# maxall41/RustSASA

Hardware: AMD Instinct MI355X
Metric: structures/sec on AF2 E. coli proteome (100 pts, 1.4 A probe) (higher is better)
Workload: dtype f32

## Files before the change

### rustsasa_amd/csrc/context.cpp

```cpp
#include "engine_internal.h"

namespace rsasa {

const char *tuning_env(const char *name)
{
    static const bool on = [] { const char *v = std::getenv("RSASA_TUNING"); return v && std::atoi(v) != 0; }();
    return on ? std::getenv(name) : nullptr;
}

void generate_sphere_points(size_t n, float *x, float *y, float *z)
{
    const float pi = 3.14159274101257324219f;
    const float angle_increment = (2.0f * pi) * 1.618034f;
    const float inv_n = 1.0f / (float)n;
    for (size_t i = 0; i < n; i++) {
        const float fi = (float)i;
        const float t = fi * inv_n;
        const float inclination = acosf(1.0f - 2.0f * t);
        const float azimuth = angle_increment * fi;
        const float si = sinf(inclination);
        x[i] = si * cosf(azimuth);
        y[i] = si * sinf(azimuth);
        z[i] = cosf(inclination);
    }
// ... 284 lines not shown

int rsasa_context::Workspace::reserve_sorted(rsasa_context *ctx, size_t N, size_t cell_words, bool with_id)
{
    int rc;
    has_id = with_id;
    if ((rc = reserve(ctx, sid_sorted, std::max<size_t>(N, 1) * 4))) return rc;
    if ((rc = reserve(ctx, rank_of, std::max<size_t>(N, 1) * 4))) return rc;
    if ((rc = reserve(ctx, cells, cell_words * 4))) return rc;
    if ((rc = reserve(ctx, sorted_xyzr, std::max<size_t>(N, 1) * 16))) return rc;
    if ((rc = reserve(ctx, sorted_orig, std::max<size_t>(N, 1) * 4))) return rc;
    if (has_id && (rc = reserve(ctx, sorted_id32, std::max<size_t>(N, 1) * 4))) return rc;
    return RSASA_OK;
}

void rsasa_context::Workspace::sorted_view(BatchView &v) const
{
    v.sid_sorted = (uint32_t *)sid_sorted.p;
    v.cell_of = (uint32_t *)cell_of.p;
    v.rank_of = (uint32_t *)rank_of.p;
    v.cells = (uint32_t *)cells.p;
    v.sorted_xyzr = (float4 *)sorted_xyzr.p;
    v.sorted_orig = (uint32_t *)sorted_orig.p;
    v.sorted_id32 = has_id ? (uint32_t *)sorted_id32.p : nullptr;
}

int rsasa_context::Workspace::reserve_grid(rsasa_context *ctx, size_t N, size_t S, size_t n_seg_all, uint64_t &capacity, bool has_tail,
                                           bool with_id)
{
    int rc;
    if (capacity == 0) capacity = std::max<uint64_t>(1u << 16, 20ull * N + 512ull * S);
    capacity = std::min<uint64_t>(capacity, 0xFFFFFFF0ull);
    cell_capacity = capacity;
    window_capacity = (uint32_t)std::min<uint64_t>(2 * cell_capacity / kWindowCells + S + 1, 0x7FFFFFFFull);
    if ((rc = reserve(ctx, segments, std::max<size_t>(n_seg_all, 1) * sizeof(Segment)))) return rc;
    if ((rc = reserve(ctx, acc, std::max<size_t>(S, 1) * sizeof(StructAcc)))) return rc;
    if ((rc = reserve(ctx, grids, std::max<size_t>(S, 1) * sizeof(StructGrid)))) return rc;
    if ((rc = reserve(ctx, grid_sums, (std::max<size_t>(S, 1) + 255) / 256 * 32))) return rc;
    if (has_tail && (rc = reserve(ctx, cell_of, std::max<size_t>(N, 1) * 4))) return rc;
    if ((rc = reserve(ctx, windows, (size_t)window_capacity * sizeof(uint4)))) return rc;
    if ((rc = reserve(ctx, scan_sums, kScanBlocks * 4))) return rc;
    if ((rc = reserve(ctx, status, sizeof(BatchStatus)))) return rc;
    return reserve_sorted(ctx, N, (size_t)(cell_capacity + 1 + 3), with_id);
}

void rsasa_context::Workspace::grid_view(BatchView &v) const
{
    sorted_view(v);
    v.segments = (const Segment *)segments.p;
    v.acc = (StructAcc *)acc.p;
    v.grids = (StructGrid *)grids.p;
    v.grid_sums = (GridSums *)grid_sums.p;
    v.cell_capacity = cell_capacity;
    v.windows = (uint4 *)windows.p;
    v.window_capacity = window_capacity;
    v.scan_block_sums = (uint32_t *)scan_sums.p;
    v.status = (BatchStatus *)status.p;
}

int rsasa_context::Workspace::reserve_occlusion(rsasa_context *ctx, const Lattice &lat, size_t N, bool with_id, bool bitmaps,
                                                bool own_values)
{
    int rc;
    keep_ids = with_id && !occlusion_uses_mx(ctx->tuning, lat, (uint32_t)N);
    id_bitmaps = bitmaps;
    ids_seg_words = bitmaps ? (uint32_t)((N + 2047) / 2048) : 0u;
    own_atom_sasa = own_values;
    if ((rc = reserve(ctx, deferred_list, std::max<size_t>(N, 1) * 4))) return rc;
    if ((rc = reserve(ctx, claim, kClaimBytes))) return rc;
    if (id_bitmaps && (rc = reserve(ctx, ids_seg, 2 * (size_t)ids_seg_words * 4 + 16))) return rc;
    if (keep_ids && (rc = reserve(ctx, sorted_id, std::max<size_t>(N, 1) * 8))) return rc;
    if (own_atom_sasa && (rc = reserve(ctx, atom_sasa, std::max<size_t>(N, 1) * 4))) return rc;
    return RSASA_OK;
}

void rsasa_context::Workspace::occlusion_view(BatchView &v) const
{
    v.deferred_list = (uint32_t *)deferred_list.p;
    v.claim = (uint32_t *)claim.p;
    v.ids_seg = id_bitmaps ? (uint32_t *)ids_seg.p : nullptr;
    v.ids_seg_words = ids_seg_words;
    v.sorted_id = keep_ids ? (uint64_t *)sorted_id.p : nullptr;
    if (own_atom_sasa) v.atom_sasa = (float *)atom_sasa.p;
}

namespace rsasa {

int grid_input_error(rsasa_context *ctx, const BatchStatus &stt)
// ... 37 lines not shown
    if (n_seg_all * sizeof(Segment) > hs.h_segments.cap) {
        if (hs.h_segments.p) RS_HIP(ctx, hipStreamSynchronize(pd.stream));
        RS_HIP(ctx, hs.h_segments.regrow((n_seg_all + n_seg_all / 2 + 64) * sizeof(Segment)));
    }
    Segment *h_segments = static_cast<Segment *>(hs.h_segments.p);
    write_segments(bt.structure_offsets_host, S, h_segments, reinterpret_cast<uint32_t *>(h_segments + n_seg));

    const bool has_id = bt.id != nullptr;
    if ((rc = W.reserve_grid(ctx, N, S, n_seg_all, ctx->cell_capacity, has_tail, has_id))) return rc;
    if ((rc = W.reserve_occlusion(ctx, lat, N, has_id, has_id, !bt.out_atom_sasa))) return rc;
    const bool keep_ids = W.keep_ids;
    if (keep_ids && pd.id32) return fail(ctx, RSASA_ERR_INTERNAL, "folded ids on a batch the per-atom kernels take");

    if (n_seg_all)
        RS_HIP(ctx, hipMemcpyAsync(W.segments.p, h_segments, n_seg_all * sizeof(Segment),
                                   hipMemcpyHostToDevice, st));

    BatchView v{};
    v.x = bt.x; v.y = bt.y; v.z = bt.z; v.radius = bt.radius; v.id = bt.id;
    v.id32 = pd.id32;
    v.ids_check = (has_id && !pd.ids_needed_known && !keep_ids && !tuning_env("RSASA_NO_ID_CHECK")) ? 1u : 0u;
    hs.ids_check = v.ids_check != 0u;
    v.large_sids = reinterpret_cast<const uint32_t *>((const Segment *)W.segments.p + n_seg);
    v.n_large = (uint32_t)n_large;
    v.ids_tables = ctx->ids_unordered_hint ? 1u : 0u;
    v.radius8 = pd.radius8;
    v.radius_table = pd.radius_table;
    v.residue_offsets = bt.residue_offsets;
    v.n_atoms = (uint32_t)N; v.n_structures = (uint32_t)S; v.n_residues = (uint32_t)R;
    v.n_segments = (uint32_t)n_seg;
    v.probe = pd.probe;
    v.atom_sasa = bt.out_atom_sasa;
    W.grid_view(v);
    W.occlusion_view(v);
    v.residue_sasa = (R && bt.residue_offsets) ? bt.out_residue_sasa : nullptr;
    v.neighbor_counts = bt.out_neighbor_counts;

    if (ctx->timing) RS_HIP(ctx, hipEventRecord(W.ev[0], st));
    launch_grid_prepare(v, st);
    rsasa_context::Workspace &other = ctx->ws[pd.ws ^ 1];
    const bool chain = other.occ_recorded && !tuning_env("RSASA_FREE_OVERLAP");
    const bool overlap = ctx->overlap_tail && has_tail;
    if (overlap && (rc = ensure_side_stream(ctx))) return rc;
    if (overlap) {
        launch_sort_lds(v, st);
        RS_HIP(ctx, hipEventRecord(ctx->ev_fork, st));
        RS_HIP(ctx, hipStreamWaitEvent(ctx->side_stream, ctx->ev_fork, 0));
        launch_sort_tail(v, ctx->side_stream);
        RS_HIP(ctx, hipEventRecord(ctx->ev_join, ctx->side_stream));
        if (ctx->timing) RS_HIP(ctx, hipEventRecord(W.ev[1], st));
        if (chain) RS_HIP(ctx, hipStreamWaitEvent(st, other.ev_occ, 0));
        if (ctx->timing) RS_HIP(ctx, hipEventRecord(W.ev[2], st));
        launch_occlusion(v, lat, ctx->tuning, kOccHead, st);
        RS_HIP(ctx, hipStreamWaitEvent(st, ctx->ev_join, 0));
        launch_occlusion(v, lat, ctx->tuning, kOccRest, st);
    } else {
        launch_sort_lds(v, st);
        if (has_tail) launch_sort_tail(v, st);
        if (ctx->timing) RS_HIP(ctx, hipEventRecord(W.ev[1], st));
        OcclusionChain oc;
        oc.wait = chain ? other.ev_occ : nullptr;
        oc.start = ctx->timing ? W.ev[2] : nullptr;
        oc.done = W.ev_occ;
        oc.expect_ids_dropped = ctx->ids_drop_hint;
        oc.solo = pd.solo_ok && v.ids_check != 0u;
        launch_occlusion(v, lat, ctx->tuning, kOccAll, st, &oc);
// ... 3 lines not shown
    if (ctx->timing) RS_HIP(ctx, hipEventRecord(W.ev[3], st));
    launch_residue_sums(v, st);
    if (ctx->timing) RS_HIP(ctx, hipEventRecord(W.ev[4], st));
    RS_HIP(ctx, hipMemcpyAsync(hs.h_status.p, W.status.p, sizeof(BatchStatus),
                               hipMemcpyDeviceToHost, st));
    RS_HIP(ctx, hipGetLastError());
    return RSASA_OK;
}

int wait_one(rsasa_context *ctx, Pending &pd)
{
    if (!pd.active) return RSASA_OK;
    rsasa_context::Workspace &W = ctx->ws[pd.ws];
    for (;;) {
        hipError_t e = hipStreamSynchronize(pd.stream);
        if (e != hipSuccess) {
            pd.active = false;
            return fail(ctx, RSASA_ERR_HIP, "hipStreamSynchronize", e);
        }
        const BatchStatus stt = ctx->slot[pd.ws].status();
        int rc = grid_verdict(ctx, stt, pd.attempts, ctx->cell_capacity);
        const bool solo_missed = rc == RSASA_OK && ctx->slot[pd.ws].ids_check && (stt.ids_unordered & 2u) != 0u;
        if (rc == kGridAgain) {
            pd.attempts++;
        } else if (solo_missed && pd.solo_ok) {
            ctx->ids_drop_hint = false;
            ctx->ids_unordered_hint = (stt.ids_unordered & 1u) != 0u;
            pd.solo_ok = false;
        } else {
            if (solo_missed) {
                rc = fail(ctx, RSASA_ERR_INTERNAL, "a launch pair reports the id-less launch's verdict");
            } else if (rc == RSASA_OK) {
                ctx->tuning.deferred_hint = stt.deferred;
                if (ctx->slot[pd.ws].ids_check) {
                    ctx->ids_drop_hint = !stt.ids_needed;
                    ctx->ids_unordered_hint = (stt.ids_unordered & 1u) != 0u;
                    ctx->ids_kept_structures.store(stt.ids_needed, std::memory_order_relaxed);
                    if (!stt.ids_needed) ctx->ids_dropped.fetch_add(1, std::memory_order_relaxed);
                }
                if (ctx->timing) {
                    float g = 0, o = 0, a = 0, t = 0;
                    (void)hipEventElapsedTime(&g, W.ev[0], W.ev[1]);
                    (void)hipEventElapsedTime(&o, W.ev[2], W.ev[3]);
                    (void)hipEventElapsedTime(&a, W.ev[3], W.ev[4]);
                    (void)hipEventElapsedTime(&t, W.ev[0], W.ev[4]);
                    ctx->timings = rsasa_timings_t{g, o, a, t, stt.grid_cells, pd.batch.n_atoms, stt.deferred};
                    ctx->timings_valid = true;
                }
            }
            pd.active = false;
            return rc;
        }
        if ((rc = enqueue_batch(ctx, pd, ctx->slot[pd.ws]))) {
            pd.active = false;
            return rc;
        }
    }
}

int wait_oldest(rsasa_context *ctx)
{
    if (ctx->n_pending == 0) return RSASA_OK;
    const int rc = wait_one(ctx, ctx->pending[ctx->head]);
    ctx->head ^= 1;
    ctx->n_pending--;
    return rc;
// ... 388 lines not shown
```

### rustsasa_amd/csrc/device_types.h

```cpp
#pragma once
#include <hip/hip_runtime.h>
#include <stdint.h>

namespace rsasa {

struct StructGrid {
    float min_x, min_y, min_z;
    float inv_cell;
    uint32_t dim_x, dim_y, dim_z;
    uint32_t cell_base;
    float max_r;
    float cell_size;
    uint32_t n_cells;
    uint32_t atom_begin;
    uint32_t n_atoms;
    uint32_t sorted_base;
    uint32_t in_lds;
    uint32_t odd_radii;
};
static_assert(sizeof(StructGrid) == 64, "StructGrid layout");

struct StructAcc {
    int min_x, min_y, min_z;
    int max_x, max_y, max_z;
// ... 41 lines not shown
inline uint32_t mx_tab_tiles(uint32_t n_points) { return n_points <= 96u ? 6u : n_points <= 112u ? 7u : 8u; }
inline uint32_t mx_tab_floats(uint32_t n_points) { return n_points > 128u ? 0u : 4u * (16u * mx_tab_tiles(n_points) + 16u) + 2u * 16u * mx_tab_tiles(n_points); }

struct GridSums {
    unsigned long long cells_s, cells_l, atoms_s, atoms_l;
};

struct BatchView {
    const float *x, *y, *z, *radius;
    const uint64_t *id;
    const uint32_t *id32;
    const uint8_t *radius8;
    const float *radius_table;
    const uint32_t *residue_offsets;
    uint32_t n_atoms, n_structures, n_residues, n_segments;
    float probe;
    uint32_t ids_check;
    const uint32_t *large_sids;
    uint32_t n_large;
    uint32_t ids_tables;
    const Segment *segments;
    StructAcc *acc;
    StructGrid *grids;
    uint32_t *sid_sorted;
    uint32_t *cell_of, *rank_of;
    uint32_t *deferred_list;
    uint32_t *claim;
    uint32_t *ids_seg;
    uint32_t ids_seg_words;
    uint32_t *cells;
    uint64_t cell_capacity;
    uint4 *windows;
    uint32_t window_capacity;
    uint32_t *scan_block_sums;
    GridSums *grid_sums;
    float4 *sorted_xyzr;
    uint32_t *sorted_orig;
    uint64_t *sorted_id;
    uint32_t *sorted_id32;
    BatchStatus *status;
    float *atom_sasa;
    float *residue_sasa;
    uint32_t *neighbor_counts;
    uint32_t *defer_flag;
    float max_r_override = __builtin_nanf("");
};

struct NbInfo {
    unsigned long long total;
    unsigned long long max_k;
    unsigned long long spill_entries;
    unsigned long long spill_atoms;
    unsigned long long spill_cursor;
    unsigned long long spill_recs;
    unsigned long long mismatch;
    unsigned long long pad;
};
static_assert(sizeof(NbInfo) == 64, "NbInfo layout");
struct NbKey {
    unsigned long long key;
    float thr;
    uint32_t pad;
};
struct NbSpillRec {
    unsigned long long off, base;
    uint32_t k, pad;
// ... 64 lines not shown
    kOccHead = 1,
    kOccRest = 2,
};
struct OcclusionChain {
    hipEvent_t wait = nullptr, start = nullptr, done = nullptr;
    bool expect_ids_dropped = true;
    bool solo = false;
};
void launch_occlusion(const BatchView &b, const Lattice &lat, const OcclusionTuning &tune,
                      OcclusionPart part, hipStream_t stream, const OcclusionChain *chain = nullptr);
bool occlusion_uses_mx(const OcclusionTuning &tune, const Lattice &lat, uint32_t n_atoms);
void launch_occlusion_deferred(const BatchView &b, const Lattice &lat, hipStream_t stream);
void launch_residue_sums(const BatchView &b, hipStream_t stream);
void launch_neighbor_count(const NbArgs &a, hipStream_t stream);
void launch_neighbor_fill(const NbArgs &a, uint64_t spill_atoms, hipStream_t stream);
void launch_accessible_points(const PtArgs &a, hipStream_t stream);
void launch_exposure_vectors(const ExArgs &e, hipStream_t stream);
void launch_contact_points(const CtArgs &c, hipStream_t stream);
void launch_neighbor_scan(const NbArgs &a, hipStream_t stream);
void launch_group_order(const GpArgs &g, hipStream_t stream);
void launch_group_points(const GpArgs &g, hipStream_t stream);
void launch_unpack_atoms(const void *records, uint32_t n_atoms, float *x, float *y, float *z, float *r, uint64_t *id,
                         const void *hdr_src, void *hdr_dst, uint32_t hdr_bytes, hipStream_t stream);
void launch_expand_frames(const float *xyz, const float *radius, const uint64_t *id,
                          const uint32_t *res_off, uint32_t n_atoms, uint32_t n_frames, uint32_t res_stride,
                          float *x, float *y, float *z, float *r, uint64_t *id_out,
                          uint32_t *res_out, hipStream_t stream);

constexpr uint32_t kSegmentAtoms = 4096;
constexpr uint32_t kScanBlocks = 1024;
constexpr uint32_t kWindowCells = 36864;
constexpr uint32_t kIdSlotsSmall = 8192, kIdAtomsSmall = 4096, kIdSlotsLarge = 73728, kIdAtomsLarge = 55296;
constexpr uint32_t kLdsMaxAtoms = 65536;

__host__ __device__ inline uint32_t grid_group_shift(uint32_t n_atoms, uint32_t n_cells)
{
    const float per_cell = (float)n_atoms / (float)(n_cells ? n_cells : 1u);
    return per_cell >= 1.0f ? 0u : per_cell >= 0.6f ? 1u : per_cell >= 0.3f ? 2u : 3u;
}
__host__ __device__ constexpr uint32_t lds_cell_slots(uint32_t n_cells) { return (n_cells + 1u + 7u) & ~7u; }
__host__ __device__ constexpr uint32_t grid_windows(uint32_t n_cells) { return (n_cells + kWindowCells - 1u) / kWindowCells; }

}
```

### rustsasa_amd/csrc/engine_internal.h

```cpp
#pragma once
#include "../../include/rustsasa_amd.h"

#include <hip/hip_runtime.h>

#include <algorithm>
#include <chrono>
#include <atomic>
#include <cmath>
#include <cstdio>
#include <cstdlib>
#include <cstring>
#include <condition_variable>
#include <deque>
#include <map>
#include <memory>
#include <mutex>
#include <thread>
#include <new>
#include <string>
#include <utility>
#include <vector>

#include <pthread.h>
#include <sched.h>
// ... 269 lines not shown
    uint64_t next_ticket = 1;
    LinkGate gate;
    bool quit = false;
};

}

using namespace rsasa;

struct rsasa_context {
    int device = 0;
    NodeCpus node;
    Stream stream;
    std::recursive_mutex mu;
    std::string last_error;
    int simd_width = 8;
    bool timing = false;
    bool small_path = true;
    bool overlap_tail = false;
    Stream side_stream;
    Event ev_fork, ev_join;
    rsasa_timings_t timings{};
    bool timings_valid = false;

    struct Workspace {
        DeviceBuffer segments, acc, grids, grid_sums, sid_sorted, deferred_list, cell_of, rank_of, cells, windows, scan_sums,
            sorted_xyzr, sorted_orig, sorted_id, sorted_id32, status, atom_sasa, claim, ids_seg;
        Event ev[5];
        Event ev_occ;
        bool occ_recorded = false;
        uint64_t cell_capacity = 0;
        uint32_t window_capacity = 0, ids_seg_words = 0;
        bool has_id = false, keep_ids = false, id_bitmaps = false, own_atom_sasa = false;

        int reserve_sorted(rsasa_context *ctx, size_t N, size_t cell_words, bool has_id);
        void sorted_view(BatchView &v) const;
        int reserve_grid(rsasa_context *ctx, size_t N, size_t S, size_t n_seg_all, uint64_t &cell_capacity, bool has_tail, bool has_id);
        void grid_view(BatchView &v) const;
        int reserve_occlusion(rsasa_context *ctx, const Lattice &lat, size_t N, bool has_id, bool id_bitmaps, bool own_atom_sasa);
        void occlusion_view(BatchView &v) const;
    } ws[2];
    static constexpr int kInFlight = 2;
    Stream stream2;
    DeviceBuffer in_x, in_y, in_z, in_r, in_id, in_res, out_res, out_k;
    static constexpr int kSlots = 8;
    struct MoreSlot { DeviceBuffer x, y, z, r, id, res, atom_sasa, out_res; } more[kSlots - 1];
    DeviceBuffer in_pack[kSlots];
    PinnedBlock h_pack;
    FoldPool *fold_pool = nullptr;
    RadiusCodec radius_codec;
    Stream copy_stream;
    Stream d2h_stream;
    Event ev_copy[kSlots];
    Event ev_d2h[kSlots];
    PinnedBlock h_out[kSlots];
    DeviceBuffer small_in, small_out;
    PinnedBlock h_small;
    DeviceBuffer tr_xyz, tr_r, tr_id, tr_res;
    struct HostSlot {
        PinnedBlock h_segments;
        PinnedBlock h_status;
        PinnedBlock h_res;
        const BatchStatus &status() const { return *static_cast<const BatchStatus *>(h_status.p); }
        bool ids_check = false;
    } slot[kSlots];
    std::atomic<uint64_t> ids_dropped{0};
    std::atomic<uint64_t> ids_kept_structures{0};
    bool ids_drop_hint = true;
    bool ids_unordered_hint = false;
    Event ev_done[kSlots];
    uint64_t cell_capacity = 0;

    std::map<std::pair<size_t, int>, LatticeEntry> lattices;
    Pending pending[2];
    int head = 0, n_pending = 0;
    OcclusionTuning tuning;
    Event ev_link;
    Event tr_ev[8][4];
    LinkGate *link_gate = nullptr;
    uint64_t link_ticket = 0;
    int own_queues = 0;
    size_t stream_sub_batches = 0;
    struct HostStream *host_stream = nullptr;
    std::atomic<int> combine_wait_us{-1};
    Workspace nb_ws;
    DeviceBuffer nb_x, nb_y, nb_z, nb_r, nb_id, nb_map, nb_counts, nb_offsets, nb_parts, nb_info, nb_entries, nb_spill, nb_recs;
    PinnedBlock nb_host;
    uint64_t nb_cell_capacity = 0;
    DeviceBuffer pt_masks, pt_sasa, pt_lattice;
    size_t pt_lattice_points = 0;
    DeviceBuffer ex_vectors, ex_free;
    DeviceBuffer ct_covered, ct_exclusive;
    DeviceBuffer gp_group, gp_sorted, gp_sorted_group, gp_own, gp_nrows, gp_offsets, gp_groups, gp_buried, gp_only, gp_self_free,
        gp_free;
};

namespace rsasa {

int fail(rsasa_context *ctx, int code, const char *what, hipError_t e = hipSuccess);

struct DeviceGuard {
// ... 129 lines not shown
```

### rustsasa_amd/csrc/host_batch.cpp

```cpp
#include "engine_internal.h"

namespace {

bool small_grid(const float mn_in[3], const float mx_in[3], float max_r, float probe, uint32_t n_atoms,
                StructGrid *out)
{
    const float cell = probe + max_r;
    const float inv = 1.0f / cell;
    if (!(cell > 0.0f) || !(inv < INFINITY) || !(cell < INFINITY)) return false;
    StructGrid g{};
    unsigned long long nc = 1;
    uint32_t d[3];
    const float mn[3] = {mn_in[0] - cell, mn_in[1] - cell, mn_in[2] - cell};
    const float mx[3] = {mx_in[0] + cell, mx_in[1] + cell, mx_in[2] + cell};
    for (int k = 0; k < 3; k++) {
        const float e = ceilf((mx[k] - mn[k]) * inv);
        if (!(e >= 0.0f) || e >= 2147483648.0f) return false;
        d[k] = (uint32_t)e + 1u;
        nc *= d[k];
        if (nc > 64ull * kWindowCells) return false;
    }
    g.min_x = mn[0]; g.min_y = mn[1]; g.min_z = mn[2];
    g.inv_cell = inv;
    g.dim_x = d[0]; g.dim_y = d[1]; g.dim_z = d[2];
// ... 113 lines not shown
    const auto t_begin = std::chrono::steady_clock::now();
    const size_t S = l.S, N = l.N, W = l.W, R = l.R;
    BatchStatus stt{};
    stt.total_cells = l.tail_begin;
    stt.tail_cell_begin = l.tail_begin;
    stt.tail_atom_base = (uint32_t)N;
    stt.n_windows = (uint32_t)W;
    std::memcpy(h, &stt, sizeof stt);
    std::memcpy(h + l.o_grid, grids, S * sizeof(StructGrid));
    if (W) std::memcpy(h + l.o_win, windows, W * sizeof(uint4));
    hipStream_t st = ctx->stream;
    char *d = (char *)ctx->small_in.p, *dout = (char *)ctx->small_out.p;
    const bool single = S == 1 && N <= kSingleAtoms && !zero_copy;
    if (zero_copy)
        launch_unpack_atoms(records, (uint32_t)N, (float *)(d + l.o_x), (float *)(d + l.o_y), (float *)(d + l.o_z), (float *)(d + l.o_r),
                            l.has_id ? (uint64_t *)(d + l.o_id) : nullptr, h, d, (uint32_t)l.o_x, st);
    else if (!single) RS_HIP(ctx, hipMemcpyAsync(d, h, l.in_bytes, hipMemcpyHostToDevice, st));
    const char *src = single ? h : d;

    BatchView v{};
    v.x = (const float *)(src + l.o_x); v.y = (const float *)(src + l.o_y); v.z = (const float *)(src + l.o_z);
    v.radius = (const float *)(src + l.o_r);
    v.id = l.has_id ? (const uint64_t *)(src + l.o_id) : nullptr;
    v.residue_offsets = R ? (const uint32_t *)(src + l.o_res) : nullptr;
    v.n_atoms = (uint32_t)N; v.n_structures = (uint32_t)S; v.n_residues = (uint32_t)R;
    v.probe = l.probe;
    v.grids = (StructGrid *)(d + l.o_grid);
    v.status = (BatchStatus *)d;
    ctx->ws[0].sorted_view(v);
    ctx->ws[0].occlusion_view(v);
    v.cell_capacity = l.tail_begin + 8;
    v.windows = (uint4 *)(d + l.o_win);
    v.window_capacity = (uint32_t)W;
    char *outp = single || zero_copy ? hout : dout;
    v.atom_sasa = (float *)(outp + l.o_oa);
    v.residue_sasa = R ? (float *)(outp + l.o_or) : nullptr;
    uint32_t *flag = reinterpret_cast<uint32_t *>(h + 56);
    *flag = 0u;
    v.defer_flag = single || zero_copy ? flag : nullptr;
    if (single) launch_sort_single(v, SingleJob{grids[0], stt}, st);
    else launch_sort_lds(v, st);
    launch_occlusion(v, lat, ctx->tuning, kOccAll, st);
    launch_residue_sums(v, st);
    if (!single && !zero_copy) RS_HIP(ctx, hipMemcpyAsync(hout, dout, l.out_bytes, hipMemcpyDeviceToHost, st));
    RS_HIP(ctx, hipGetLastError());
    const auto t_queued = std::chrono::steady_clock::now();
    RS_HIP(ctx, hipStreamSynchronize(st));
    if (zero_copy) {
        const auto t_done = std::chrono::steady_clock::now();
        g_small_trace_ns[0].fetch_add((uint64_t)std::chrono::duration_cast<std::chrono::nanoseconds>(t_queued - t_begin).count(), std::memory_order_relaxed);
        g_small_trace_ns[1].fetch_add((uint64_t)std::chrono::duration_cast<std::chrono::nanoseconds>(t_done - t_queued).count(), std::memory_order_relaxed);
    }
    if ((single || zero_copy) && *flag) {
        launch_occlusion_deferred(v, lat, st);
        launch_residue_sums(v, st);
        RS_HIP(ctx, hipGetLastError());
        RS_HIP(ctx, hipStreamSynchronize(st));
    }
    return RSASA_OK;
}

int run_small_host_batch(rsasa_context *ctx, const SmallSource &in, const uint32_t *so, size_t S,
                         float probe, size_t n_points, float *out_atom, const uint32_t *ro, size_t R,
                         float *out_res)
{
    if (S == 0 || S > kSmallStructures || so[0] != 0 || n_points == 0 || n_points > (1u << 24) ||
// ... 444 lines not shown
            bt.x = dev_x[0];
            bt.y = dev_y[0];
            bt.z = dev_z[0];
            bt.radius = (const float *)br[0]->p;
            bt.id = id && !drop_ids[0] ? (const uint64_t *)bi[0]->p : nullptr;
            bt.structure_offsets_host = so[0].data();
            bt.n_structures = n_structures;
            bt.n_atoms = na;
            bt.residue_offsets = nr ? (const uint32_t *)bo[0]->p : nullptr;
            bt.n_residues = nr;
            bt.out_atom_sasa = (float *)oa[0]->p;
            bt.out_residue_sasa = nr ? (float *)orr[0]->p : nullptr;
            bt.out_neighbor_counts = nullptr;
            if ((rc = batch_enqueue(ctx, &bt, probe_radius, n_points, nullptr, false))) return rc;
            if ((rc = rsasa_batch_wait(ctx))) return rc;
        }
        if ((rc = copy_out(0))) return rc;
        if ((rc = drain(0))) return rc;
        RS_HIP(ctx, hipStreamSynchronize(ctx->d2h_stream));
        return RSASA_OK;
    }

    struct Attempt {
        uint64_t need_cells = 0;
        int err = RSASA_OK;
        bool used[kSlots] = {};
    };

    void check(int k, Attempt &at)
    {
        const BatchStatus stt = ctx->slot[k].status();
        if (!at.err) at.err = grid_input_error(ctx, stt);
        if (stt.overflow) at.need_cells = std::max<uint64_t>(at.need_cells, stt.total_cells);
        else ctx->tuning.deferred_hint = stt.deferred;
        if (!stt.overflow && ctx->slot[k].ids_check) {
            ctx->ids_drop_hint = !stt.ids_needed;
            ctx->ids_unordered_hint = (stt.ids_unordered & 1u) != 0u;
            ctx->ids_kept_structures.store(stt.ids_needed, std::memory_order_relaxed);
            if (!stt.ids_needed) ctx->ids_dropped.fetch_add(1, std::memory_order_relaxed);
        }
    }

    void submit_coding_jobs()
    {
        if (!(fold_ids || code_radii)) return;
        if (code_radii) ctx->radius_codec.reset();
        for (size_t c = 0; c < n_sub; c++) {
            const size_t a0 = structure_offsets[cut[c]], na = atoms_of(c);
            char *blk = (char *)ctx->h_pack.p + pack[c].base;
            IdOrder order;
            ids_matter[c].store(0);
            if (fold_ids && check_ids) {
                order.starts = structure_offsets + cut[c];
                order.n_starts = cut[c + 1] - cut[c];
                order.first = (uint32_t)a0;
                order.ids_matter = &ids_matter[c];
            }
            fold_job[c] = ctx->fold_pool->submit(fold_ids ? id + a0 : nullptr,
                                                 fold_ids ? reinterpret_cast<uint32_t *>(blk + pack[c].o_id) : nullptr, na,
                                                 radius + a0, code_radii ? reinterpret_cast<uint8_t *>(blk + pack[c].o_r8) : nullptr,
                                                 code_radii ? &ctx->radius_codec : nullptr, order);
        }
        fold_drain.pool = ctx->fold_pool;
        fold_drain.last = fold_job[n_sub - 1];
    }

    int launch_sub_batch(size_t c, Attempt &at)
// ... 450 lines not shown
```

### rustsasa_amd/csrc/kernels.hip

```cpp
#include "device_utils.h"

#include <algorithm>

namespace rsasa {

namespace {


__global__ void k_init_acc(StructAcc *acc, uint32_t n_structures, BatchStatus *status, uint32_t ids_needed, uint32_t *ids_seg, uint32_t ids_seg_words)
{
    uint32_t s = blockIdx.x * blockDim.x + threadIdx.x;
    for (uint32_t i = s; ids_seg && i < 2u * ids_seg_words; i += gridDim.x * blockDim.x) ids_seg[i] = 0u;
    if (s == 0) {
        status->overflow = 0;
        status->grid_too_large = 0;
        status->bad_input = 0;
        status->deferred = 0;
        status->total_cells = 0;
        status->tail_cell_begin = 0;
        status->tail_atom_base = 0;
        status->n_windows = 0;
        status->grid_cells = 0;
        status->ids_needed = ids_needed;
        status->ids_unordered = 0;
// ... 247 lines not shown
                              n_windows > b.window_capacity) ? 1u : 0u;
    }
}

__global__ __launch_bounds__(256) void k_grid_bases(BatchView b)
{
    __shared__ unsigned long long part[4][4];
    const uint32_t s = blockIdx.x * blockDim.x + threadIdx.x;
    uint32_t ncells = 0, na = 0;
    bool in_lds = false;
    if (s < b.n_structures) {
        ncells = b.grids[s].n_cells;
        na = b.grids[s].n_atoms;
        in_lds = b.grids[s].in_lds != 0u;
    }
    const uint32_t slots = lds_cell_slots(ncells), n_win = grid_windows(ncells);
    const unsigned long long own = na | ((unsigned long long)n_win << 32);
    GridSums v = {in_lds ? slots : 0u, in_lds ? 0u : ncells, in_lds ? own : 0ull, in_lds ? 0u : na};
    (void)block_scan_sums<4>(v, part);
    if (s < b.n_structures) {
        const GridSums base = b.grid_sums[blockIdx.x];
        const unsigned long long cb = in_lds ? base.cells_s + v.cells_s - slots
                                             : b.status->tail_cell_begin + base.cells_l + v.cells_l - ncells;
        const unsigned long long as = base.atoms_s + v.atoms_s - own;
        b.grids[s].cell_base = (uint32_t)(cb > 0xFFFFFFFFull ? 0xFFFFFFFFull : cb);
        b.grids[s].sorted_base = in_lds ? (uint32_t)as : (uint32_t)(b.status->tail_atom_base + base.atoms_l + v.atoms_l - na);
        if (in_lds && !batch_aborted(b.status)) {
            const uint32_t w0 = (uint32_t)(as >> 32);
            for (uint32_t w = 0; w < n_win; w++) b.windows[w0 + w] = make_uint4(s, w, b.grids[s].atom_begin, na);
        }
    }
}

constexpr uint32_t kSortWindowThreads = 1024u;
template <bool SINGLE>
__global__ __launch_bounds__(kSortWindowThreads, SINGLE ? 4 : 8) void k_sort_window(BatchView b, SingleJob single)
{
    constexpr uint32_t kThreads = kSortWindowThreads;
    constexpr int kSlots = 8;
    constexpr uint32_t kStage = kWindowCells * 2u / 32u;
    constexpr uint32_t kPer = ((kWindowCells / 2u + kThreads - 1u) / kThreads) | 1u;
    __shared__ __attribute__((aligned(16))) uint32_t s_cnt[kWindowCells / 2 + 4 + kPer + 3];
    __shared__ uint32_t smem32[16];
    __shared__ uint32_t s_below;
    uint32_t s, c0, a0, n_at;
    StructGrid g;
    if (SINGLE) {
        s = 0;
        c0 = blockIdx.x * kWindowCells;
        g = single.grid;
        a0 = g.atom_begin; n_at = g.n_atoms;
        if (blockIdx.x == 0 && threadIdx.x == 0) {
            b.grids[0] = g;
            *b.status = single.status;
        }
    } else {
        const uint4 job = b.windows[blockIdx.x];
        if (batch_aborted(b.status) || blockIdx.x >= b.status->n_windows) return;
        s = job.x;
        c0 = job.y * kWindowCells;
        a0 = job.z; n_at = job.w;
    }
    const uint32_t tid = threadIdx.x;
    const uint32_t a1 = a0 + n_at;
    const float *__restrict__ px = b.x, *__restrict__ py = b.y, *__restrict__ pz = b.z;
    auto pr = [&](uint32_t i) { return load_radius(b.radius, b.radius8, b.radius_table, i); };
    const uint32_t *__restrict__ pid32 = b.id32;
    const uint64_t *__restrict__ pid = pid32 ? reinterpret_cast<const uint64_t *>(pid32) : b.id;
    uint32_t *__restrict__ rank_of = b.rank_of;
    uint4 *stage = reinterpret_cast<uint4 *>(s_cnt);
    float x[kSlots], y[kSlots], z[kSlots];
    float kr[SINGLE ? kSlots : 1];
    uint64_t kid[SINGLE ? kSlots : 1];
#pragma unroll
    for (int k = 0; k < kSlots; k++) {
        x[k] = y[k] = z[k] = 0.f;
        if (SINGLE) { kr[k] = 0.f; kid[k] = 0ull; }
        if (kThreads * k < n_at) {
            const uint32_t i = min(a0 + tid + kThreads * k, a1 - 1u);
            x[k] = px[i]; y[k] = py[i]; z[k] = pz[i];
            if (SINGLE) {
                kr[k] = pr(i);
                if (pid) kid[k] = load_id(b.id, pid32, i);
            }
        }
    }
    if (!SINGLE) g = b.grids[s];
    if (!SINGLE && b.ids_check && (g.odd_radii & 2u) == 0u) pid = nullptr;
    const uint32_t dim_xy = g.dim_x * g.dim_y;
    const uint32_t n_cells = min(kWindowCells, g.n_cells - c0), n_words = (n_cells + 1u) >> 1;
    const bool last_window = c0 + n_cells == g.n_cells;
    for (uint32_t i = tid; i < ((n_words / kPer + 1u) * kPer + 3u) / 4u; i += kThreads) stage[i] = make_uint4(0u, 0u, 0u, 0u);
    if (tid == 0) s_below = 0;
    constexpr uint32_t kNotMine = 0xFFFFFFFFu;
    uint32_t rcell[kSlots], rpos[kSlots];
    uint32_t below = 0;
#pragma unroll
    for (int k = 0; k < kSlots; k++) {
        uint32_t cx, cy, cz;
        cell_coords(g, x[k], y[k], z[k], cx, cy, cz);
        const bool live = a0 + tid + kThreads * k < a1;
        const uint32_t c = cx + cy * g.dim_x + cz * dim_xy;
        rcell[k] = live ? c - c0 : 0xFFFFFFFFu;
        rpos[k] = kNotMine;
        if (c0) below += (uint32_t)__popcll(ballot64(live && c < c0));
    }
    const uint32_t a_rest = a0 + kThreads * kSlots;
    __syncthreads();
#pragma unroll
    for (int k = 0; k < kSlots; k++) {
        const uint32_t lc = rcell[k];
        if (lc < n_cells) atomicAdd(&s_cnt[lc >> 1], 1u << ((lc & 1u) * 16u));
    }
    for (uint32_t i0 = a_rest + tid; i0 < a1; i0 += 4u * kThreads) {
        float xx[4], yy[4], zz[4];
#pragma unroll
        for (int k = 0; k < 4; k++) {
            const uint32_t i = min(i0 + kThreads * k, a1 - 1u);
            xx[k] = px[i]; yy[k] = py[i]; zz[k] = pz[i];
        }
// ... 137 lines not shown
            idr[k] = pid ? load_id(b.id, pid32, i) : 0ull;
        }
#pragma unroll
        for (int k = 0; k < 4; k++) {
            const uint32_t i = i0 + kThreads * k;
            uint32_t cx, cy, cz;
            cell_coords(g, v[k].x, v[k].y, v[k].z, cx, cy, cz);
            const uint32_t lc = cx + cy * g.dim_x + cz * dim_xy - c0;
            if (i < a1 && lc < n_cells) {
                const uint32_t rel = pos[k] - placed;
                if (rel < kStage) {
                    stage[2u * rel] = __builtin_bit_cast(uint4, v[k]);
                    stage[2u * rel + 1u] = make_uint4(i, fold_id(idr[k]), (uint32_t)idr[k], (uint32_t)(idr[k] >> 32));
                } else {
                    const uint32_t p = g.sorted_base + pos[k];
                    b.sorted_xyzr[p] = v[k];
                    b.sorted_orig[p] = i;
                    if (pid) { if (b.sorted_id) b.sorted_id[p] = idr[k]; b.sorted_id32[p] = fold_id(idr[k]); }
                }
            }
        }
    }
    __syncthreads();
    for (uint32_t j = tid; j < n_staged; j += kThreads) {
        const uint4 q = stage[2u * j + 1u];
        b.sorted_xyzr[out0 + j] = __builtin_bit_cast(float4, stage[2u * j]);
        b.sorted_orig[out0 + j] = q.x;
        if (pid) {
            b.sorted_id32[out0 + j] = q.y;
            if (b.sorted_id) b.sorted_id[out0 + j] = (uint64_t)q.z | ((uint64_t)q.w << 32);
        }
    }
    for (uint32_t j = tid; j < total; j += kThreads) b.sid_sorted[out0 + j] = s;
}


__global__ __launch_bounds__(256) void k_zero_cells(BatchView b)
{
    if (batch_aborted(b.status)) return;
    const uint64_t n4 = (b.status->total_cells + 1 + 3) / 4;
    uint4 *c4 = reinterpret_cast<uint4 *>(b.cells);
    for (uint64_t i = b.status->tail_cell_begin / 4 + (uint64_t)blockIdx.x * blockDim.x + threadIdx.x; i < n4;
         i += (uint64_t)gridDim.x * blockDim.x)
        c4[i] = make_uint4(0u, 0u, 0u, 0u);
}

constexpr uint32_t kSegmentParts = 4;

__global__ __launch_bounds__(256) void k_cell_hist(BatchView b)
{
    if (batch_aborted(b.status)) return;
    const Segment seg = b.segments[blockIdx.x / kSegmentParts];
    const StructGrid g = b.grids[seg.sid];
    if (g.in_lds) return;
    const uint32_t part = kSegmentAtoms / kSegmentParts, p0 = seg.begin + (blockIdx.x % kSegmentParts) * part;
    for (uint32_t i = p0 + threadIdx.x; i < min(seg.end, p0 + part); i += blockDim.x) {
        uint32_t cx, cy, cz;
        cell_coords(g, b.x[i], b.y[i], b.z[i], cx, cy, cz);
        const uint32_t cell = g.cell_base + cx + cy * g.dim_x + cz * g.dim_x * g.dim_y;
        b.cell_of[i] = cell;
        b.rank_of[i] = atomicAdd(&b.cells[cell], 1u);
    }
}

__device__ __forceinline__ void scan_range(const BatchView &b, uint64_t &begin, uint64_t &end)
{
// ... 61 lines not shown
    const Segment seg = b.segments[blockIdx.x / kSegmentParts];
    const uint32_t s = seg.sid;
    if (b.grids[s].in_lds) return;
    const uint32_t part = kSegmentAtoms / kSegmentParts, p0 = seg.begin + (blockIdx.x % kSegmentParts) * part;
    for (uint32_t i = p0 + threadIdx.x; i < min(seg.end, p0 + part); i += blockDim.x) {
        const uint32_t pos = b.cells[b.cell_of[i]] + b.rank_of[i];
        b.sorted_xyzr[pos] = make_float4(b.x[i], b.y[i], b.z[i], load_radius(b.radius, b.radius8, b.radius_table, i));
        b.sorted_orig[pos] = i;
        b.sid_sorted[pos] = s;
        if (b.sorted_id32 && !(b.ids_check && (b.grids[s].odd_radii & 2u) == 0u)) { const uint64_t v = load_id(b.id, b.id32, i); if (b.sorted_id) b.sorted_id[pos] = v; b.sorted_id32[pos] = fold_id(v); }
    }
}

__global__ __launch_bounds__(256) void k_residue_sums(BatchView b)
{
    if (batch_aborted(b.status)) return;
    uint32_t k = blockIdx.x * blockDim.x + threadIdx.x;
    if (k >= b.n_residues) return;
    float total = 0.0f;
    for (uint32_t i = b.residue_offsets[k], e = b.residue_offsets[k + 1]; i < e; i++)
        total += b.atom_sasa[i];
    b.residue_sasa[k] = total;
}

}

void launch_grid_prepare(const BatchView &b, hipStream_t stream)
{
    hipLaunchKernelGGL(k_init_acc, dim3(cdiv(b.n_structures > 0 ? b.n_structures : 1, 256)), dim3(256), 0, stream,
                       b.acc, b.n_structures, b.status, b.ids_check ? 0u : 1u, b.ids_check ? b.ids_seg : nullptr, b.ids_seg_words);
    if (b.n_segments)
        hipLaunchKernelGGL(k_bounds, dim3(b.n_segments), dim3(256), 0, stream, b);
    const uint32_t n_parts = cdiv(b.n_structures > 0 ? b.n_structures : 1, 256);
    hipLaunchKernelGGL(k_grid_params, dim3(n_parts), dim3(256), 0, stream, b);
    if (n_parts <= 256) hipLaunchKernelGGL(k_grid_scan<1>, dim3(1), dim3(64), 0, stream, b, n_parts);
    else hipLaunchKernelGGL(k_grid_scan<16>, dim3(1), dim3(1024), 0, stream, b, n_parts);
    hipLaunchKernelGGL(k_grid_bases, dim3(n_parts), dim3(256), 0, stream, b);
    if (b.ids_check && b.ids_tables && b.n_structures) {
        hipLaunchKernelGGL((k_ids_distinct<kIdSlotsSmall, 256u, false>), dim3(b.n_structures), dim3(256), 0, stream, b);
        if (b.n_large)
            hipLaunchKernelGGL((k_ids_distinct<kIdSlotsLarge, 1024u, true>), dim3(b.n_large), dim3(1024), 0, stream, b);
    }
    if (b.ids_check && b.ids_seg && b.n_structures) hipLaunchKernelGGL(k_ids_segments, dim3(n_parts), dim3(256), 0, stream, b);
}

void launch_sort_lds(const BatchView &b, hipStream_t stream)
{
    if (b.window_capacity) hipLaunchKernelGGL(k_sort_window<false>, dim3(b.window_capacity), dim3(kSortWindowThreads), 0, stream, b, SingleJob{});
}

void launch_sort_single(const BatchView &b, const SingleJob &job, hipStream_t stream)
{
    const uint32_t n_win = grid_windows(job.grid.n_cells);
    if (n_win) hipLaunchKernelGGL(k_sort_window<true>, dim3(n_win), dim3(kSortWindowThreads), 0, stream, b, job);
}

void launch_sort_tail(const BatchView &b, hipStream_t stream)
{
    hipLaunchKernelGGL(k_zero_cells, dim3(2048), dim3(256), 0, stream, b);
    if (b.n_segments)
        hipLaunchKernelGGL(k_cell_hist, dim3(b.n_segments * kSegmentParts), dim3(256), 0, stream, b);
    hipLaunchKernelGGL(k_scan_reduce, dim3(kScanBlocks), dim3(256), 0, stream, b);
    hipLaunchKernelGGL(k_scan_block_sums, dim3(1), dim3(kScanBlocks), 0, stream, b);
    hipLaunchKernelGGL(k_scan_apply, dim3(kScanBlocks), dim3(256), 0, stream, b);
    if (b.n_segments)
        hipLaunchKernelGGL(k_scatter, dim3(b.n_segments * kSegmentParts), dim3(256), 0, stream, b);
}

__global__ __launch_bounds__(256) void k_expand_frames(const float *xyz, const float *radius,
                                                       const uint64_t *id, const uint32_t *res_off,
                                                       uint32_t n_atoms, uint32_t n_frames,
                                                       uint32_t res_stride, float *x, float *y, float *z,
                                                       float *r, uint64_t *id_out, uint32_t *res_out)
{
    const uint32_t n_res = res_stride;
    const uint64_t total = (uint64_t)n_atoms * n_frames;
    const uint64_t i = (uint64_t)blockIdx.x * blockDim.x + threadIdx.x;
    if (i < total) {
        const uint32_t a = (uint32_t)(i % n_atoms);
        x[i] = xyz[3 * i + 0];
        y[i] = xyz[3 * i + 1];
        z[i] = xyz[3 * i + 2];
        r[i] = radius[a];
        if (id) id_out[i] = id[a];
    }
    const uint64_t total_res = (uint64_t)n_res * n_frames;
    if (res_off && i <= total_res) {
// ... 47 lines not shown
```

Before: 1.323 million.

## Fuse grid placement into one block and size sort-window launch from previous batch

For batches up to a structure-count threshold, the three-kernel grid params/scan/bases sequence, and optionally the id-segment bitmap kernel, is replaced by a single 1024-thread block kernel. This removes several launches and inter-kernel dependencies. The LDS sort-window launch is also sized from the window count the previous batch reported, plus a margin, instead of the worst-case capacity. A small persistent 'rest' kernel covers any windows beyond that launch size. This cuts idle block launches, at the cost of a serial single-block placement pass and an extra launch whenever the hint underestimates.

New measurement: 1.315 million. Within noise of the previous version (-0.6%).

```diff
diff --git a/rustsasa_amd/csrc/context.cpp b/rustsasa_amd/csrc/context.cpp
--- a/rustsasa_amd/csrc/context.cpp
+++ b/rustsasa_amd/csrc/context.cpp
@@ -340,6 +340,8 @@
     capacity = std::min<uint64_t>(capacity, 0xFFFFFFF0ull);
     cell_capacity = capacity;
     window_capacity = (uint32_t)std::min<uint64_t>(2 * cell_capacity / kWindowCells + S + 1, 0x7FFFFFFFull);
+    const char *place_max = tuning_env("RSASA_PLACE_ONE_MAX");
+    place_one = S <= (place_max ? (size_t)std::strtoull(place_max, nullptr, 10) : (size_t)kPlaceOneStructures);
     if ((rc = reserve(ctx, segments, std::max<size_t>(n_seg_all, 1) * sizeof(Segment)))) return rc;
     if ((rc = reserve(ctx, acc, std::max<size_t>(S, 1) * sizeof(StructAcc)))) return rc;
     if ((rc = reserve(ctx, grids, std::max<size_t>(S, 1) * sizeof(StructGrid)))) return rc;
@@ -361,6 +363,8 @@
     v.cell_capacity = cell_capacity;
     v.windows = (uint4 *)windows.p;
     v.window_capacity = window_capacity;
+    v.window_launch = window_capacity;
+    v.place_one = place_one ? 1u : 0u;
     v.scan_block_sums = (uint32_t *)scan_sums.p;
     v.status = (BatchStatus *)status.p;
 }
@@ -464,6 +468,7 @@
     v.probe = pd.probe;
     v.atom_sasa = bt.out_atom_sasa;
     W.grid_view(v);
+    v.window_launch = sort_window_launch(ctx->windows_hint, v.window_capacity);
     W.occlusion_view(v);
     v.residue_sasa = (R && bt.residue_offsets) ? bt.out_residue_sasa : nullptr;
     v.neighbor_counts = bt.out_neighbor_counts;
@@ -533,6 +538,7 @@
                 rc = fail(ctx, RSASA_ERR_INTERNAL, "a launch pair reports the id-less launch's verdict");
             } else if (rc == RSASA_OK) {
                 ctx->tuning.deferred_hint = stt.deferred;
+                ctx->windows_hint = stt.n_windows;
                 if (ctx->slot[pd.ws].ids_check) {
                     ctx->ids_drop_hint = !stt.ids_needed;
                     ctx->ids_unordered_hint = (stt.ids_unordered & 1u) != 0u;
diff --git a/rustsasa_amd/csrc/device_types.h b/rustsasa_amd/csrc/device_types.h
--- a/rustsasa_amd/csrc/device_types.h
+++ b/rustsasa_amd/csrc/device_types.h
@@ -97,6 +97,8 @@
     uint64_t cell_capacity;
     uint4 *windows;
     uint32_t window_capacity;
+    uint32_t window_launch;
+    uint32_t place_one;
     uint32_t *scan_block_sums;
     GridSums *grid_sums;
     float4 *sorted_xyzr;
@@ -227,6 +229,15 @@
 constexpr uint32_t kWindowCells = 36864;
 constexpr uint32_t kIdSlotsSmall = 8192, kIdAtomsSmall = 4096, kIdSlotsLarge = 73728, kIdAtomsLarge = 55296;
 constexpr uint32_t kLdsMaxAtoms = 65536;
+constexpr uint32_t kPlaceThreads = 1024, kPlaceOneStructures = 16384;
+constexpr uint32_t kWindowLaunchFloor = 256, kWindowRestLaunch = 128;
+inline uint32_t sort_window_launch(uint32_t hint, uint32_t capacity)
+{
+    if (hint == 0xFFFFFFFFu) return capacity;
+    uint64_t want = (uint64_t)hint + hint / 8u + 64u;
+    if (want < kWindowLaunchFloor) want = kWindowLaunchFloor;
+    return want < capacity ? (uint32_t)want : capacity;
+}
 
 __host__ __device__ inline uint32_t grid_group_shift(uint32_t n_atoms, uint32_t n_cells)
 {
diff --git a/rustsasa_amd/csrc/engine_internal.h b/rustsasa_amd/csrc/engine_internal.h
--- a/rustsasa_amd/csrc/engine_internal.h
+++ b/rustsasa_amd/csrc/engine_internal.h
@@ -325,6 +325,7 @@
         uint64_t cell_capacity = 0;
         uint32_t window_capacity = 0, ids_seg_words = 0;
         bool has_id = false, keep_ids = false, id_bitmaps = false, own_atom_sasa = false;
+        bool place_one = false;
 
         int reserve_sorted(rsasa_context *ctx, size_t N, size_t cell_words, bool has_id);
         void sorted_view(BatchView &v) const;
@@ -360,6 +361,7 @@
     std::atomic<uint64_t> ids_dropped{0};
     std::atomic<uint64_t> ids_kept_structures{0};
     bool ids_drop_hint = true;
+    uint32_t windows_hint = 0xFFFFFFFFu;
     bool ids_unordered_hint = false;
     Event ev_done[kSlots];
     uint64_t cell_capacity = 0;
diff --git a/rustsasa_amd/csrc/host_batch.cpp b/rustsasa_amd/csrc/host_batch.cpp
--- a/rustsasa_amd/csrc/host_batch.cpp
+++ b/rustsasa_amd/csrc/host_batch.cpp
@@ -169,6 +169,7 @@
     v.cell_capacity = l.tail_begin + 8;
     v.windows = (uint4 *)(d + l.o_win);
     v.window_capacity = (uint32_t)W;
+    v.window_launch = (uint32_t)W;
     char *outp = single || zero_copy ? hout : dout;
     v.atom_sasa = (float *)(outp + l.o_oa);
     v.residue_sasa = R ? (float *)(outp + l.o_or) : nullptr;
@@ -679,7 +680,10 @@
         const BatchStatus stt = ctx->slot[k].status();
         if (!at.err) at.err = grid_input_error(ctx, stt);
         if (stt.overflow) at.need_cells = std::max<uint64_t>(at.need_cells, stt.total_cells);
-        else ctx->tuning.deferred_hint = stt.deferred;
+        else {
+            ctx->tuning.deferred_hint = stt.deferred;
+            ctx->windows_hint = stt.n_windows;
+        }
         if (!stt.overflow && ctx->slot[k].ids_check) {
             ctx->ids_drop_hint = !stt.ids_needed;
             ctx->ids_unordered_hint = (stt.ids_unordered & 1u) != 0u;
diff --git a/rustsasa_amd/csrc/kernels.hip b/rustsasa_amd/csrc/kernels.hip
--- a/rustsasa_amd/csrc/kernels.hip
+++ b/rustsasa_amd/csrc/kernels.hip
@@ -303,8 +303,97 @@
     }
 }
 
+template <bool IDS_SEG>
+__global__ __launch_bounds__(kPlaceThreads) void k_grid_place(BatchView b)
+{
+    constexpr int NW = kPlaceThreads / kWave;
+    __shared__ unsigned long long part[NW][4];
+    __shared__ unsigned long long s_grid_cells;
+    const uint32_t S = b.n_structures, tid = threadIdx.x;
+    if (tid == 0) s_grid_cells = 0;
+    __syncthreads();
+    GridSums v = {0, 0, 0, 0};
+    unsigned long long n_cells = 0;
+    bool bad = false, too_large = false;
+    for (uint32_t s = tid; s < S; s += kPlaceThreads) {
+        const StructGrid g = make_grid(b.acc[s], b.probe, b.max_r_override, bad, too_large);
+        b.grids[s] = g;
+        if (g.in_lds) { v.cells_s += lds_cell_slots(g.n_cells); v.atoms_s += g.n_atoms | ((unsigned long long)grid_windows(g.n_cells) << 32); }
+        else { v.cells_l += g.n_cells; v.atoms_l += g.n_atoms; }
+        n_cells += g.n_cells;
+    }
+    if (bad) b.status->bad_input = 1u;
+    if (too_large) b.status->grid_too_large = 1u;
+#pragma unroll
+    for (int d = kWave / 2; d > 0; d >>= 1) n_cells += __shfl_xor(n_cells, d, kWave);
+    if (lane_id() == 0 && n_cells) atomicAdd(&s_grid_cells, n_cells);
+    const GridSums tot = block_scan_sums<NW>(v, part);
+    const bool any_too_large = __syncthreads_or(too_large ? 1 : 0) != 0;
+    const unsigned long long tail_begin = (tot.cells_s / 2ull + 1023ull) & ~1023ull;
+    const unsigned long long total = tail_begin + tot.cells_l;
+    const unsigned long long n_windows = tot.atoms_s >> 32;
+    const uint32_t tail_atom_base = (uint32_t)tot.atoms_s;
+    const bool overflow = total > b.cell_capacity || total > 0xFFFFFFF0ull || tot.cells_s > 0xFFFFFFF0ull || n_windows > b.window_capacity;
+    if (tid == 0) {
+        b.status->total_cells = total;
+        b.status->tail_cell_begin = tail_begin;
+        b.status->tail_atom_base = tail_atom_base;
+        b.status->n_windows = (uint32_t)min(n_windows, 0xFFFFFFFFull);
+        b.status->overflow = overflow ? 1u : 0u;
+        b.status->grid_cells = s_grid_cells;
+    }
+    const bool aborted = overflow || any_too_large;
+    GridSums carry = {0, 0, 0, 0};
+    for (uint32_t s0 = 0; s0 < S; s0 += kPlaceThreads) {
+        const uint32_t s = s0 + tid;
+        uint32_t ncells = 0, na = 0, atom_begin = 0, odd = 0;
+        bool in_lds = false;
+        if (s < S) {
+            ncells = b.grids[s].n_cells;
+            na = b.grids[s].n_atoms;
+            in_lds = b.grids[s].in_lds != 0u;
+            atom_begin = b.grids[s].atom_begin;
+            odd = b.grids[s].odd_radii;
+        }
+        const uint32_t slots = lds_cell_slots(ncells), n_win = grid_windows(ncells);
+        const unsigned long long own = na | ((unsigned long long)n_win << 32);
+        GridSums x = {in_lds ? slots : 0u, in_lds ? 0u : ncells, in_lds ? own : 0ull, in_lds ? 0u : na};
+        const GridSums trip = block_scan_sums<NW>(x, part);
+        if (s < S) {
+            const unsigned long long cb = in_lds ? carry.cells_s + x.cells_s - slots : tail_begin + carry.cells_l + x.cells_l - ncells;
+            const unsigned long long as = carry.atoms_s + x.atoms_s - own;
+            const uint32_t sorted_base = in_lds ? (uint32_t)as : (uint32_t)(tail_atom_base + carry.atoms_l + x.atoms_l - na);
+            b.grids[s].cell_base = (uint32_t)(cb > 0xFFFFFFFFull ? 0xFFFFFFFFull : cb);
+            b.grids[s].sorted_base = sorted_base;
+            if (in_lds && !aborted) {
+                const uint32_t w0 = (uint32_t)(as >> 32);
+                for (uint32_t w = 0; w < n_win; w++) b.windows[w0 + w] = make_uint4(s, w, atom_begin, na);
+            }
+            if (IDS_SEG && na) {
+                uint32_t *bits = b.ids_seg + ((odd & 2u) ? 0u : b.ids_seg_words);
+                const uint32_t p0 = sorted_base >> 6, p1 = (sorted_base + na - 1u) >> 6;
+                for (uint32_t w = p0 >> 5; w <= (p1 >> 5) && w < b.ids_seg_words; w++) {
+                    const uint32_t lo = max(p0, w << 5) & 31u, hi = min(p1, (w << 5) + 31u) & 31u;
+                    atomicOr(&bits[w], (0xFFFFFFFFu >> (31u - hi)) & (0xFFFFFFFFu << lo));
+                }
+            }
+        }
+        carry.cells_s += trip.cells_s; carry.cells_l += trip.cells_l;
+        carry.atoms_s += trip.atoms_s; carry.atoms_l += trip.atoms_l;
+    }
+}
+
 constexpr uint32_t kSortWindowThreads = 1024u;
-template <bool SINGLE>
+__device__ __forceinline__ uint32_t uniform32(uint32_t v) { return (uint32_t)__builtin_amdgcn_readfirstlane((int)v); }
+__device__ __forceinline__ StructGrid load_grid_uniform(const StructGrid *p)
+{
+    struct Words { uint32_t w[sizeof(StructGrid) / 4]; };
+    Words u = __builtin_bit_cast(Words, *p);
+#pragma unroll
+    for (uint32_t k = 0; k < sizeof(StructGrid) / 4; k++) u.w[k] = uniform32(u.w[k]);
+    return __builtin_bit_cast(StructGrid, u);
+}
+template <bool SINGLE, bool REST = false>
 __global__ __launch_bounds__(kSortWindowThreads, SINGLE ? 4 : 8) void k_sort_window(BatchView b, SingleJob single)
 {
     constexpr uint32_t kThreads = kSortWindowThreads;
@@ -314,6 +403,14 @@
     __shared__ __attribute__((aligned(16))) uint32_t s_cnt[kWindowCells / 2 + 4 + kPer + 3];
     __shared__ uint32_t smem32[16];
     __shared__ uint32_t s_below;
+    uint32_t n_win = 0;
+    uint4 first = make_uint4(0u, 0u, 0u, 0u);
+    if (!SINGLE) {
+        if (!REST) first = b.windows[blockIdx.x];
+        if (batch_aborted(b.status)) return;
+        n_win = b.status->n_windows;
+    }
+    for (uint32_t w = (REST ? b.window_launch : 0u) + blockIdx.x; SINGLE || w < n_win; w += gridDim.x) {
     uint32_t s, c0, a0, n_at;
     StructGrid g;
     if (SINGLE) {
@@ -326,11 +423,11 @@
             *b.status = single.status;
         }
     } else {
-        const uint4 job = b.windows[blockIdx.x];
-        if (batch_aborted(b.status) || blockIdx.x >= b.status->n_windows) return;
-        s = job.x;
-        c0 = job.y * kWindowCells;
-        a0 = job.z; n_at = job.w;
+        if (REST && w != b.window_launch + blockIdx.x) __syncthreads();
+        const uint4 job = REST ? b.windows[w] : first;
+        s = REST ? uniform32(job.x) : job.x;
+        c0 = (REST ? uniform32(job.y) : job.y) * kWindowCells;
+        a0 = REST ? uniform32(job.z) : job.z; n_at = REST ? uniform32(job.w) : job.w;
     }
     const uint32_t tid = threadIdx.x;
     const uint32_t a1 = a0 + n_at;
@@ -356,7 +453,7 @@
             }
         }
     }
-    if (!SINGLE) g = b.grids[s];
+    if (!SINGLE) g = REST ? load_grid_uniform(&b.grids[s]) : b.grids[s];
     if (!SINGLE && b.ids_check && (g.odd_radii & 2u) == 0u) pid = nullptr;
     const uint32_t dim_xy = g.dim_x * g.dim_y;
     const uint32_t n_cells = min(kWindowCells, g.n_cells - c0), n_words = (n_cells + 1u) >> 1;
@@ -560,6 +657,8 @@
         }
     }
     for (uint32_t j = tid; j < total; j += kThreads) b.sid_sorted[out0 + j] = s;
+    if (!REST) break;
+    }
 }
 
 
@@ -687,27 +786,39 @@
     if (b.n_segments)
         hipLaunchKernelGGL(k_bounds, dim3(b.n_segments), dim3(256), 0, stream, b);
     const uint32_t n_parts = cdiv(b.n_structures > 0 ? b.n_structures : 1, 256);
-    hipLaunchKernelGGL(k_grid_params, dim3(n_parts), dim3(256), 0, stream, b);
-    if (n_parts <= 256) hipLaunchKernelGGL(k_grid_scan<1>, dim3(1), dim3(64), 0, stream, b, n_parts);
-    else hipLaunchKernelGGL(k_grid_scan<16>, dim3(1), dim3(1024), 0, stream, b, n_parts);
-    hipLaunchKernelGGL(k_grid_bases, dim3(n_parts), dim3(256), 0, stream, b);
+    const bool segments_fused = b.place_one && b.ids_check && b.ids_seg && b.n_structures && !b.ids_tables;
+    if (b.place_one) {
+        if (segments_fused) hipLaunchKernelGGL(k_grid_place<true>, dim3(1), dim3(kPlaceThreads), 0, stream, b);
+        else hipLaunchKernelGGL(k_grid_place<false>, dim3(1), dim3(kPlaceThreads), 0, stream, b);
+    } else {
+        hipLaunchKernelGGL(k_grid_params, dim3(n_parts), dim3(256), 0, stream, b);
+        if (n_parts <= 256) hipLaunchKernelGGL(k_grid_scan<1>, dim3(1), dim3(64), 0, stream, b, n_parts);
+        else hipLaunchKernelGGL(k_grid_scan<16>, dim3(1), dim3(1024), 0, stream, b, n_parts);
+        hipLaunchKernelGGL(k_grid_bases, dim3(n_parts), dim3(256), 0, stream, b);
+    }
     if (b.ids_check && b.ids_tables && b.n_structures) {
         hipLaunchKernelGGL((k_ids_distinct<kIdSlotsSmall, 256u, false>), dim3(b.n_structures), dim3(256), 0, stream, b);
         if (b.n_large)
             hipLaunchKernelGGL((k_ids_distinct<kIdSlotsLarge, 1024u, true>), dim3(b.n_large), dim3(1024), 0, stream, b);
     }
-    if (b.ids_check && b.ids_seg && b.n_structures) hipLaunchKernelGGL(k_ids_segments, dim3(n_parts), dim3(256), 0, stream, b);
+    if (b.ids_check && b.ids_seg && b.n_structures && !segments_fused) hipLaunchKernelGGL(k_ids_segments, dim3(n_parts), dim3(256), 0, stream, b);
 }
 
 void launch_sort_lds(const BatchView &b, hipStream_t stream)
 {
-    if (b.window_capacity) hipLaunchKernelGGL(k_sort_window<false>, dim3(b.window_capacity), dim3(kSortWindowThreads), 0, stream, b, SingleJob{});
+    BatchView v = b;
+    v.window_launch = std::min(b.window_launch, b.window_capacity);
+    if (!v.window_launch) return;
+    hipLaunchKernelGGL((k_sort_window<false, false>), dim3(v.window_launch), dim3(kSortWindowThreads), 0, stream, v, SingleJob{});
+    if (v.window_launch < b.window_capacity)
+        hipLaunchKernelGGL((k_sort_window<false, true>), dim3(std::min(kWindowRestLaunch, b.window_capacity - v.window_launch)),
+                           dim3(kSortWindowThreads), 0, stream, v, SingleJob{});
 }
 
 void launch_sort_single(const BatchView &b, const SingleJob &job, hipStream_t stream)
 {
     const uint32_t n_win = grid_windows(job.grid.n_cells);
-    if (n_win) hipLaunchKernelGGL(k_sort_window<true>, dim3(n_win), dim3(kSortWindowThreads), 0, stream, b, job);
+    if (n_win) hipLaunchKernelGGL((k_sort_window<true, false>), dim3(n_win), dim3(kSortWindowThreads), 0, stream, b, job);
 }
 
 void launch_sort_tail(const BatchView &b, hipStream_t stream)
```
